# SamsungSAILMontreal/ghn3

Hardware: AMD Instinct MI355X
Metric: predicted-params/sec (GHN fwd+bwd), ghn3xlm16, 256-node graphs (higher is better)
Workload: dtype f16; 1 GPU; ghn3xlm16 fwd+bwd, 1 synthetic 256-node graph(s) per GPU (seed 256000+), 86515016 predicted params per GPU, loss = sum of Frobenius norms of the predicted tensors; ghn_params=654365312, decoder_rows=1421, workspace_bytes=2436048640, zero_fill_bytes=2797339192, parallelism=dp1, index_mode=reference, loss=fused into the tile kernels

## Files before the change

### ghn3_amd/csrc/elementwise.hip

```cpp

#include "ghn3_internal.h"

#define MAX_DEGREE 100
#define MAX_INPUT_DIST 1000

__device__ __forceinline__ float wsum(float v) {
#pragma unroll
    for (int o = 32; o > 0; o >>= 1) v += __shfl_xor(v, o, 64);
    return v;
}

static int launch_ok(const char* what) {
    hipError_t e = hipGetLastError();
    if (e != hipSuccess) { ghn3_set_error("%s launch: %s", what, hipGetErrorString(e)); return GHN3_E_HIP; }
    return GHN3_OK;
}

__global__ __launch_bounds__(256) void graph_prologue_kernel(const int64_t* __restrict__ A, int* __restrict__ deg_in,
                                                             int* __restrict__ deg_out, int* __restrict__ dist0,
                                                             int* __restrict__ pair, int N, int V) {
    __shared__ int red[2][4];
    const int i = blockIdx.x, b = blockIdx.y;
    const int64_t* Ab = A + (size_t)b * N * N;
    int cnt_out = 0, cnt_in = 0;
// ... 450 lines not shown
                    const int c = lane + 64 * j;
                    pv[p][j] = (p < n_add && c < C) ? ar[p * add_stride + c] : 0.f;
                }
#pragma unroll
            for (int p = 0; p < LN_PLANES; ++p)
#pragma unroll
                for (int j = 0; j < LN_REG; ++j) dgv[j] += pv[p][j];
            for (int p = LN_PLANES; p < n_add; ++p)
                for (int j = 0; j < LN_REG; ++j) { const int c = lane + 64 * j; if (c < C) dgv[j] += ar[p * add_stride + c]; }
#pragma unroll
            for (int j = 0; j < LN_REG; ++j) { const int c = lane + 64 * j; if (c < C) gr[c] = dgv[j]; }
        }
#pragma unroll
        for (int j = 0; j < LN_REG; ++j) { const int c = lane + 64 * j; dgv[j] *= (c < C) ? g[c] : 0.f; }
        float s1 = 0.f, s2 = 0.f;
#pragma unroll
        for (int j = 0; j < LN_REG; ++j)
            if (lane + 64 * j < C) {
                s1 += dgv[j];
                s2 += dgv[j] * (xh[j] - mu) * rs;
            }
        s1 = wsum(s1) / (float)C;
        s2 = wsum(s2) / (float)C;
#pragma unroll
        for (int j = 0; j < LN_REG; ++j) {
            const int c = lane + 64 * j;
            if (c < C) {
                const float h = (xh[j] - mu) * rs;
                float v = rs * (dgv[j] - s1 - h * s2);
                if (rr) v += rv[j];
                dr[c] = v;
            }
        }
        return;
    }
    if (ar)
        for (int c = lane; c < C; c += 64) {
            float v = gr[c];
            for (int p = 0; p < n_add; ++p) v += ar[p * add_stride + c];
            gr[c] = v;
        }
    float s1 = 0.f, s2 = 0.f;
    for (int c = lane; c < C; c += 64) {
        const float dg = gr[c] * g[c];
        s1 += dg;
        s2 += dg * (xr[c] - mu) * rs;
    }
    s1 = wsum(s1) / (float)C;
    s2 = wsum(s2) / (float)C;
    for (int c = lane; c < C; c += 64) {
        const float xh = (xr[c] - mu) * rs;
        float v = rs * (gr[c] * g[c] - s1 - xh * s2);
        if (rr) v += rr[c];
        dr[c] = v;
    }
}
int ghn3_layernorm_bwd(float* dx, float* dy, const float* x, const float* g, const float* mean,
                       const float* rstd, const float* res, const float* add, int n_add, int64_t add_stride, int rows,
                       int C, hipStream_t s) {
    if (add && n_add <= 0) n_add = 1;
    hipLaunchKernelGGL(layernorm_bwd_kernel, dim3((rows + 3) / 4), dim3(256), 0, s, dx, dy, x, g, mean, rstd, res, add,
                       n_add, add_stride, rows, C);
    return launch_ok("layernorm_bwd");
}

__global__ __launch_bounds__(256) void ln_param_grad_kernel(float* __restrict__ dg, float* __restrict__ db,
                                                            const float* __restrict__ dy, const float* __restrict__ x,
                                                            const float* __restrict__ mean,
                                                            const float* __restrict__ rstd, int rows, int C, int accum) {
    __shared__ float sg[16][16], sb[16][16];
    const int cl = threadIdx.x & 15, rl = threadIdx.x >> 4;
    const int c = blockIdx.x * 16 + cl;
    float ag = 0.f, ab = 0.f;
    if (c < C) {
        for (int r0 = rl; r0 < rows; r0 += 16 * 8) {
            float d[8], xv[8], mu[8], rs[8];
#pragma unroll
            for (int k = 0; k < 8; ++k) {
                const int r = r0 + 16 * k;
                const bool in = r < rows;
                d[k] = in ? dy[(size_t)r * C + c] : 0.f;
                xv[k] = in ? x[(size_t)r * C + c] : 0.f;
                mu[k] = in ? mean[r] : 0.f;
                rs[k] = in ? rstd[r] : 0.f;
            }
#pragma unroll
            for (int k = 0; k < 8; ++k) { ag += d[k] * (xv[k] - mu[k]) * rs[k]; ab += d[k]; }
        }
    }
    sg[rl][cl] = ag; sb[rl][cl] = ab;
    __syncthreads();
    if (rl == 0 && c < C) {
        float g = 0.f, b = 0.f;
#pragma unroll
        for (int k = 0; k < 16; ++k) { g += sg[k][cl]; b += sb[k][cl]; }
        dg[c] = accum ? dg[c] + g : g;
        db[c] = accum ? db[c] + b : b;
    }
}
__global__ __launch_bounds__(256) void ln_param_grad_batch_kernel(float* __restrict__ gbase, const float* __restrict__ abase,
                                                                  const int64_t* __restrict__ table, int rows, int C) {
    __shared__ float sg[16][16], sb[16][16];
    const int64_t* T = table + 6 * (int64_t)blockIdx.y;
    float* dg = gbase + T[0];
    float* db = gbase + T[1];
    const float* dy = abase + T[2];
    const float* x = abase + T[3];
    const float* mean = abase + T[4];
    const float* rstd = abase + T[5];
    const int cl = threadIdx.x & 15, rl = threadIdx.x >> 4;
    const int c = blockIdx.x * 16 + cl;
    float ag = 0.f, ab = 0.f;
    if (c < C) {
        for (int r0 = rl; r0 < rows; r0 += 16 * 8) {
            float d[8], xv[8], mu[8], rs[8];
#pragma unroll
            for (int k = 0; k < 8; ++k) {
                const int r = r0 + 16 * k;
                const bool in = r < rows;
                d[k] = in ? dy[(size_t)r * C + c] : 0.f;
                xv[k] = in ? x[(size_t)r * C + c] : 0.f;
                mu[k] = in ? mean[r] : 0.f;
                rs[k] = in ? rstd[r] : 0.f;
            }
#pragma unroll
            for (int k = 0; k < 8; ++k) { ag += d[k] * (xv[k] - mu[k]) * rs[k]; ab += d[k]; }
        }
    }
    sg[rl][cl] = ag; sb[rl][cl] = ab;
    __syncthreads();
    if (rl == 0 && c < C) {
        float g = 0.f, b = 0.f;
#pragma unroll
        for (int k = 0; k < 16; ++k) { g += sg[k][cl]; b += sb[k][cl]; }
        dg[c] += g;
        db[c] += b;
    }
}
int ghn3_ln_param_grad_batch(float* gbase, const float* abase, const int64_t* table, int n_items, int rows, int C,
                             hipStream_t s) {
    if (n_items <= 0 || rows <= 0 || C <= 0) return GHN3_OK;
    hipLaunchKernelGGL(ln_param_grad_batch_kernel, dim3((C + 15) / 16, n_items), dim3(256), 0, s, gbase, abase, table, rows, C);
    return launch_ok("ln_param_grad_batch");
}

int ghn3_ln_param_grad(float* dg, float* db, const float* dy, const float* x, const float* mean, const float* rstd,
                       int rows, int C, int accum, hipStream_t s) {
    hipLaunchKernelGGL(ln_param_grad_kernel, dim3((C + 15) / 16), dim3(256), 0, s, dg, db, dy, x, mean, rstd, rows, C,
                       accum);
    return launch_ok("ln_param_grad");
}

struct RowSet { int64_t off; int32_t rows, o, i, ld, i0, _pad; };
__global__ __launch_bounds__(256) void rowset_colsum_kernel(float* __restrict__ out, const float* __restrict__ X,
                                                            const RowSet* __restrict__ sets, int n_sets, int I) {
    __shared__ float red[4][64];
    const int l = threadIdx.x & 63, rl = threadIdx.x >> 6;
    const int ip = blockIdx.x * 64 + l, op = blockIdx.y;
    float acc = 0.f;
    for (int k = 0; k < n_sets; ++k) {
        const RowSet S = sets[k];
        const int il = ip - S.i0;
        if (op >= S.o || (int)(blockIdx.x * 64 + 63) < S.i0 || (int)(blockIdx.x * 64) >= S.i0 + S.i) continue;
        if (il >= 0 && il < S.i) {
            const float* p = X + S.off + (size_t)op * S.i + il;
            for (int r0 = rl; r0 < S.rows; r0 += 4 * 8) {
                float v[8];
#pragma unroll
                for (int e = 0; e < 8; ++e) { const int r = r0 + 4 * e; v[e] = r < S.rows ? p[(size_t)r * S.ld] : 0.f; }
#pragma unroll
                for (int e = 0; e < 8; ++e) acc += v[e];
            }
        }
    }
    red[rl][l] = acc;
    __syncthreads();
    if (rl == 0 && ip < I) out[(size_t)op * I + ip] += (red[0][l] + red[1][l]) + (red[2][l] + red[3][l]);
}
int ghn3_rowset_colsum(float* out, const float* X, const void* sets, int n_sets, int O, int I, hipStream_t s) {
    if (n_sets <= 0 || O <= 0 || I <= 0) return GHN3_OK;
    hipLaunchKernelGGL(rowset_colsum_kernel, dim3((I + 63) / 64, O), dim3(256), 0, s, out, X,
                       reinterpret_cast<const RowSet*>(sets), n_sets, I);
    return launch_ok("rowset_colsum");
}

#define TILE_CHUNK 2048

__device__ __forceinline__ float norm_apply(float v, int mode, float scale) {
    if (mode == 0) return v * scale;
    if (mode == 1) return 2.f / (1.f + __expf(-0.5f * v));
    return tanhf(0.2f * v);
}
__device__ __forceinline__ float norm_grad(float v, int mode, float scale) {
    if (mode == 0) return scale;
    if (mode == 1) { float sg = 1.f / (1.f + __expf(-0.5f * v)); return sg * (1.f - sg); }
    float th = tanhf(0.2f * v);
    return 0.2f * (1.f - th * th);
}

typedef float f4u __attribute__((ext_vector_type(4), aligned(4)));
typedef unsigned short us4h __attribute__((ext_vector_type(4)));
struct SrcTable { const float* p[6]; };
struct DstTable { float* p[6]; };

struct Odo {
    int d[4];
    int T[4];
    int s[4];
    __device__ __forceinline__ void init(unsigned e, unsigned stride, int t0, int t1, int t2, int t3) {
        T[0] = t0; T[1] = t1; T[2] = t2; T[3] = t3;
        unsigned q = e;
        d[3] = q % t3; q /= t3; d[2] = q % t2; q /= t2; d[1] = q % t1; d[0] = q / t1;
        q = stride;
        s[3] = q % t3; q /= t3; s[2] = q % t2; q /= t2; s[1] = q % t1; s[0] = q / t1;
    }
    __device__ __forceinline__ void step() {
        int c = 0;
#pragma unroll
        for (int k = 3; k >= 1; --k) {
            int v = d[k] + s[k] + c;
            c = v >= T[k];
            d[k] = c ? v - T[k] : v;
        }
        d[0] += s[0] + c;
    }
};

__device__ __forceinline__ void tile_block_sumsq(float ss, float bm, float* __restrict__ sq_parts, float* __restrict__ b_parts,
                                                 const ghn3_tile_desc* __restrict__ D) {
    __shared__ float sq_red[4], mx_red[4];
    ss = wsum(ss);
#pragma unroll
    for (int o = 32; o > 0; o >>= 1) bm = fmaxf(bm, __shfl_xor(bm, o, 64));
    __syncthreads();
    if ((threadIdx.x & 63) == 0) { sq_red[threadIdx.x >> 6] = ss; mx_red[threadIdx.x >> 6] = bm; }
    __syncthreads();
    if (threadIdx.x == 0) {
        sq_parts[blockIdx.x] = (sq_red[0] + sq_red[1]) + (sq_red[2] + sq_red[3]);
        if (b_parts) {
            float f = 0.f;
            if (D->src_buf == 0 && D->mode == 0) {
                f = fabsf(D->scale);
#pragma unroll
                for (int k = 0; k < 4; ++k) f *= (float)((D->T[k] + D->E[k] - 1) / D->E[k]);
            }
            b_parts[blockIdx.x] = fmaxf(fmaxf(mx_red[0], mx_red[1]), fmaxf(mx_red[2], mx_red[3])) * f;
        }
    }
}

__global__ __launch_bounds__(256) void tile_fwd_kernel(float* __restrict__ flat, SrcTable srcs,
                                                       const ghn3_tile_desc* __restrict__ desc,
                                                       const int64_t* __restrict__ blocks, float* __restrict__ sq_parts,
                                                       float* __restrict__ b_parts) {
    extern __shared__ float tl[];
    float ss = 0.f, bm = 0.f;
    const int64_t di_raw = blocks[2 * (size_t)blockIdx.x];
    if (di_raw < 0) {
        const ghn3_tile_desc* D = desc + (~di_raw);
        const int64_t word = blocks[2 * (size_t)blockIdx.x + 1];
        const int a0 = (int)(word & 0xffffff), i0 = (int)(word >> 24);
        const int T1 = D->T[1], T3 = D->T[3], hw = D->T[2] * T3, E1 = D->E[1];
        const int ni = min(D->_pad, T1 - i0);
        const float* src = srcs.p[D->src_buf] + D->src_off + (int64_t)(a0 % D->E[0]) * D->S[0];
        const int n = ni * hw;
        const int S2 = (int)D->S[2], S3 = (int)D->S[3];
        const float inv_ni = 1.f / (float)ni, inv_t3 = 1.f / (float)T3;
        const bool vec = E1 == T1 && (ni & 3) == 0 && (S2 & 3) == 0 && (S3 & 3) == 0 &&
                         ((reinterpret_cast<uintptr_t>(src + i0)) & 15) == 0;
        if (vec) {
            const int ni4 = ni >> 2, n4 = ni4 * hw;
            const float inv_ni4 = 1.f / (float)ni4;
            constexpr int U = 4;
            for (int b0 = threadIdx.x; b0 < n4; b0 += 256 * U) {
                float4 v[U];
                int li[U];
#pragma unroll
                for (int u = 0; u < U; ++u) {
                    const int idx = b0 + 256 * u;
                    int pp = (int)((float)idx * inv_ni4);
                    int i4 = idx - pp * ni4;
                    if (i4 < 0) { i4 += ni4; --pp; } else if (i4 >= ni4) { i4 -= ni4; ++pp; }
                    int y = (int)((float)pp * inv_t3);
                    int x = pp - y * T3;
                    if (x < 0) { x += T3; --y; } else if (x >= T3) { x -= T3; ++y; }
                    li[u] = i4 * 4 * hw + pp;
                    v[u] = idx < n4 ? *reinterpret_cast<const float4*>(src + (int64_t)y * S2 + (int64_t)x * S3 + i0 + i4 * 4)
                                    : make_float4(0.f, 0.f, 0.f, 0.f);
                }
#pragma unroll
                for (int u = 0; u < U; ++u)
                    if (b0 + 256 * u < n4) {
                        tl[li[u]] = v[u].x; tl[li[u] + hw] = v[u].y; tl[li[u] + 2 * hw] = v[u].z; tl[li[u] + 3 * hw] = v[u].w;
                    }
            }
        } else {
            constexpr int U = 8;
            for (int b0 = threadIdx.x; b0 < n; b0 += 256 * U) {
                float v[U];
                int li[U];
#pragma unroll
                for (int u = 0; u < U; ++u) {
                    const int idx = b0 + 256 * u;
                    int pp = (int)((float)idx * inv_ni);
                    int i = idx - pp * ni;
                    if (i < 0) { i += ni; --pp; } else if (i >= ni) { i -= ni; ++pp; }
                    int y = (int)((float)pp * inv_t3);
                    int x = pp - y * T3;
                    if (x < 0) { x += T3; --y; } else if (x >= T3) { x -= T3; ++y; }
                    li[u] = i * hw + pp;
                    const int si = i0 + i;
                    v[u] = idx < n ? src[(int64_t)y * S2 + (int64_t)x * S3 + (E1 == T1 ? si : si % E1)] : 0.f;
                }
#pragma unroll
                for (int u = 0; u < U; ++u)
                    if (b0 + 256 * u < n) tl[li[u]] = v[u];
            }
        }
        __syncthreads();
        float* dst = flat + D->dst_off + ((int64_t)a0 * T1 + i0) * hw;
        const float scale = D->scale;
        const int nv = n & ~3;
        for (int j = threadIdx.x * 4; j < nv; j += 1024) {
            f4u o;
            o.x = tl[j] * scale; o.y = tl[j + 1] * scale; o.z = tl[j + 2] * scale; o.w = tl[j + 3] * scale;
            *reinterpret_cast<f4u*>(dst + j) = o;
            ss += (o.x * o.x + o.y * o.y) + (o.z * o.z + o.w * o.w);
            bm = fmaxf(fmaxf(bm, fmaxf(fabsf(o.x), fabsf(o.y))), fmaxf(fabsf(o.z), fabsf(o.w)));
        }
        for (int j = nv + threadIdx.x; j < n; j += 256) { const float o = tl[j] * scale; dst[j] = o; ss += o * o; bm = fmaxf(bm, fabsf(o)); }
        if (sq_parts) tile_block_sumsq(ss, bm, sq_parts, b_parts, D);
        return;
    }
    const int64_t di = di_raw;
    const unsigned start = (unsigned)blocks[2 * (size_t)blockIdx.x + 1];
// ... 702 lines not shown
                    const float4 v = *reinterpret_cast<const float4*>(p);
                    acc[0] += v.x; acc[1] += v.y; acc[2] += v.z; acc[3] += v.w;
                } else for (int k = 0; k < cnt; ++k) acc[k] += p[k];
            }
        }
        for (int k = 0; k < cnt; ++k) {
            if (OUT16) reinterpret_cast<unsigned short*>(out_)[e + k] = wire_bf16(acc[k] * scale);
            else reinterpret_cast<float*>(out_)[e + k] = acc[k] * scale;
        }
    }
}
int ghn3_rank_reduce(void* out, const void* in, int64_t per, int W, int in16, int out16, float scale, hipStream_t s) {
    if (per <= 0 || W <= 0) return GHN3_OK;
    int64_t blocks = (per / 4 + 255) / 256 + 1;
    if (blocks > 8192) blocks = 8192;
    const dim3 g((unsigned)blocks), b(256);
    if (in16 && out16) hipLaunchKernelGGL((rank_reduce_kernel<true, true>), g, b, 0, s, out, in, per, W, scale);
    else if (in16) hipLaunchKernelGGL((rank_reduce_kernel<true, false>), g, b, 0, s, out, in, per, W, scale);
    else if (out16) hipLaunchKernelGGL((rank_reduce_kernel<false, true>), g, b, 0, s, out, in, per, W, scale);
    else hipLaunchKernelGGL((rank_reduce_kernel<false, false>), g, b, 0, s, out, in, per, W, scale);
    return launch_ok("rank_reduce");
}

__global__ __launch_bounds__(256) void transpose32_kernel(float* __restrict__ dst, const float* __restrict__ src, int rows, int cols,
                                                          int ld_src, int ld_dst, int64_t sb, int64_t db) {
    __shared__ float t[64][65];
    const float* S = src + (int64_t)blockIdx.z * sb;
    float* D = dst + (int64_t)blockIdx.z * db;
    const int r0 = blockIdx.y * 64, c0 = blockIdx.x * 64;
    const int tx = threadIdx.x & 15, ty = threadIdx.x >> 4;
    for (int i = ty; i < 64; i += 16) {
        const int r = r0 + i, c = c0 + tx * 4;
        float4 v = {0.f, 0.f, 0.f, 0.f};
        if (r < rows) {
            if (c + 3 < cols && ((ld_src & 3) == 0) && ((reinterpret_cast<uintptr_t>(S) & 15) == 0)) v = *reinterpret_cast<const float4*>(S + (int64_t)r * ld_src + c);
            else { float e[4] = {0.f, 0.f, 0.f, 0.f}; for (int k = 0; k < 4; ++k) if (c + k < cols) e[k] = S[(int64_t)r * ld_src + c + k]; v = {e[0], e[1], e[2], e[3]}; }
        }
        t[i][tx * 4] = v.x; t[i][tx * 4 + 1] = v.y; t[i][tx * 4 + 2] = v.z; t[i][tx * 4 + 3] = v.w;
    }
    __syncthreads();
    for (int i = ty; i < 64; i += 16) {
        const int c = c0 + i, r = r0 + tx * 4;
        if (c >= cols) continue;
        float e[4] = {t[tx * 4][i], t[tx * 4 + 1][i], t[tx * 4 + 2][i], t[tx * 4 + 3][i]};
        if (r + 3 < rows && ((ld_dst & 3) == 0) && ((reinterpret_cast<uintptr_t>(D) & 15) == 0)) *reinterpret_cast<float4*>(D + (int64_t)c * ld_dst + r) = float4{e[0], e[1], e[2], e[3]};
        else for (int k = 0; k < 4; ++k) if (r + k < rows) D[(int64_t)c * ld_dst + r + k] = e[k];
    }
}
int ghn3_transpose32(float* dst, const float* src, int rows, int cols, int ld_src, int ld_dst, int batch, int64_t sb, int64_t db,
                     hipStream_t s) {
    if (rows <= 0 || cols <= 0 || batch <= 0) return GHN3_OK;
    if (batch > 65535 || (rows + 63) / 64 > 65535) { ghn3_set_error("transpose32: too many batches / row tiles"); return GHN3_E_LIMIT; }
    hipLaunchKernelGGL(transpose32_kernel, dim3((cols + 63) / 64, (rows + 63) / 64, batch), dim3(256), 0, s, dst, src, rows, cols,
                       ld_src, ld_dst, sb, db);
    return launch_ok("transpose32");
}

__device__ __forceinline__ unsigned short cast_f16(float x) {
    const float c = x != x ? x : __builtin_amdgcn_fmed3f(x, -65504.f, 65504.f);
    return __builtin_bit_cast(unsigned short, (_Float16)c);
}
__device__ __forceinline__ unsigned short cast_bf16(float x) {
    unsigned u = __builtin_bit_cast(unsigned, x);
    u += 0x7fffu + ((u >> 16) & 1u);
    return (unsigned short)(u >> 16);
}
__device__ __forceinline__ float bf16_back(unsigned short h) { return __builtin_bit_cast(float, (unsigned)h << 16); }
__device__ __forceinline__ float f16_back(unsigned short h) { return (float)__builtin_bit_cast(_Float16, h); }
typedef unsigned short us4 __attribute__((ext_vector_type(4)));
typedef unsigned short us8 __attribute__((ext_vector_type(8)));

struct AdamWArgs { float lr, beta1, beta2, eps, weight_decay, bias_corr1, bias_corr2_sqrt, max_norm, inv_scale; int nt; };
typedef float f32x4_nt __attribute__((ext_vector_type(4)));
__device__ __forceinline__ float4 ld4(const float* p, bool nt) {
    if (nt) { const f32x4_nt v = __builtin_nontemporal_load(reinterpret_cast<const f32x4_nt*>(p)); return make_float4(v[0], v[1], v[2], v[3]); }
    return *reinterpret_cast<const float4*>(p);
}
__device__ __forceinline__ void st4(float* p, const float4& x, bool nt) {
    if (nt) { const f32x4_nt v = {x.x, x.y, x.z, x.w}; __builtin_nontemporal_store(v, reinterpret_cast<f32x4_nt*>(p)); }
    else *reinterpret_cast<float4*>(p) = x;
}
static int adamw_nt_env() {
    static const int v = getenv("GHN3_ADAMW_NT") ? atoi(getenv("GHN3_ADAMW_NT")) != 0 : 1;
    return v;
}
template <typename MT> struct AdamWSrcT { const float* g; MT* m; MT* v; const float* sumsq; AdamWArgs a; };
typedef AdamWSrcT<float> AdamWSrc;

struct AdamWRng { unsigned key; unsigned base; };
__host__ __device__ __forceinline__ unsigned adamw_mix32(unsigned x) {
    x ^= x >> 16; x *= 0x7feb352du; x ^= x >> 15; x *= 0x846ca68bu; x ^= x >> 16;
    return x;
}
static unsigned adamw_rng_key(unsigned seed, unsigned step) { return adamw_mix32(seed * 0x9e3779b9u + step); }
__device__ __forceinline__ unsigned short bf16_stochastic(float x, unsigned r16) {
    return (unsigned short)((__builtin_bit_cast(unsigned, x) + r16) >> 16);
}
typedef unsigned u32x2_nt __attribute__((ext_vector_type(2)));
template <int NT> __device__ __forceinline__ float4 ld_m4(const float* p, bool nt) { return ld4(p, nt); }
template <int NT> __device__ __forceinline__ float4 ld_m4(const unsigned short* p, bool) {
    u32x2_nt w;
    if constexpr (NT > 0) w = __builtin_nontemporal_load(reinterpret_cast<const u32x2_nt*>(p));
    else w = *reinterpret_cast<const u32x2_nt*>(p);
    return make_float4(__builtin_bit_cast(float, w[0] << 16), __builtin_bit_cast(float, w[0] & 0xffff0000u),
                       __builtin_bit_cast(float, w[1] << 16), __builtin_bit_cast(float, w[1] & 0xffff0000u));
}
template <int NT>
__device__ __forceinline__ void st_mv4(float* m, float* v, const float4& mv, const float4& vv, bool nt, const AdamWRng&, unsigned) {
    st4(m, mv, nt); st4(v, vv, nt);
}
template <int NT>
__device__ __forceinline__ void st_mv4(unsigned short* m, unsigned short* v, const float4& mv, const float4& vv, bool,
                                       const AdamWRng& rng, unsigned idx) {
    const unsigned h0 = adamw_mix32(idx ^ rng.key), h1 = adamw_mix32((idx + 1u) ^ rng.key),
                   h2 = adamw_mix32((idx + 2u) ^ rng.key), h3 = adamw_mix32((idx + 3u) ^ rng.key);
    const u32x2_nt wm = {(unsigned)bf16_stochastic(mv.x, h0 & 0xffffu) | ((unsigned)bf16_stochastic(mv.y, h1 & 0xffffu) << 16),
                         (unsigned)bf16_stochastic(mv.z, h2 & 0xffffu) | ((unsigned)bf16_stochastic(mv.w, h3 & 0xffffu) << 16)};
    const u32x2_nt wv = {(unsigned)bf16_stochastic(vv.x, h0 >> 16) | ((unsigned)bf16_stochastic(vv.y, h1 >> 16) << 16),
                         (unsigned)bf16_stochastic(vv.z, h2 >> 16) | ((unsigned)bf16_stochastic(vv.w, h3 >> 16) << 16)};
    if constexpr (NT > 0) {
        __builtin_nontemporal_store(wm, reinterpret_cast<u32x2_nt*>(m));
        __builtin_nontemporal_store(wv, reinterpret_cast<u32x2_nt*>(v));
    } else {
        *reinterpret_cast<u32x2_nt*>(m) = wm;
        *reinterpret_cast<u32x2_nt*>(v) = wv;
    }
}
__device__ __forceinline__ float ld_m1(const float* p) { return *p; }
__device__ __forceinline__ float ld_m1(const unsigned short* p) { return bf16_back(*p); }
__device__ __forceinline__ void st_mv1(float* m, float* v, float mi, float vi, const AdamWRng&, unsigned) { *m = mi; *v = vi; }
__device__ __forceinline__ void st_mv1(unsigned short* m, unsigned short* v, float mi, float vi, const AdamWRng& rng, unsigned idx) {
    const unsigned h = adamw_mix32(idx ^ rng.key);
    *m = bf16_stochastic(mi, h & 0xffffu); *v = bf16_stochastic(vi, h >> 16);
}

__device__ __forceinline__ float nofuse(float x) { asm volatile("" : "+v"(x)); return x; }
__device__ __forceinline__ void adamw_scalars(const AdamWArgs& a, const float* sumsq, float& clip, float& step, float& decay) {
    clip = a.inv_scale;
    if (sumsq && a.max_norm > 0.f)
        clip = clip * fminf(1.f, a.max_norm / (nofuse(sqrtf(*sumsq) * a.inv_scale) + 1e-6f));
    step = a.lr / a.bias_corr1;
    decay = 1.f - nofuse(a.lr * a.weight_decay);
}
__device__ __forceinline__ void adamw_element(float& p, float g, float& m, float& v, const AdamWArgs& a, float clip,
                                              float step, float decay) {
    const float gi = g * clip;
    const float mi = __builtin_fmaf(a.beta1, m, nofuse((1.f - a.beta1) * gi));
    const float vi = __builtin_fmaf(a.beta2, v, nofuse(nofuse((1.f - a.beta2) * gi) * gi));
    m = mi; v = vi;
    const float den = nofuse(sqrtf(vi) / a.bias_corr2_sqrt) + a.eps;
    p = nofuse(p * decay) - nofuse(nofuse(step * mi) / den);
}

template <bool ADAMW, typename MT = float, int NT = -1>
__device__ __forceinline__ void cast16_body(const float* __restrict__ src, unsigned short* __restrict__ dst,
                                            const ghn3_cast_desc* __restrict__ descs, int n_desc,
                                            float* __restrict__ dbias, int total_items,
                                            const float* __restrict__ amax, const AdamWSrcT<MT>& aw,
                                            const AdamWRng& rng = AdamWRng{}) {
    __shared__ unsigned short tr[64][66];
    __shared__ float csum[16][64];
    float aw_clip = 1.f, aw_step = 0.f, aw_decay = 1.f;
    if (ADAMW) {
        if (aw.sumsq && !isfinite(*aw.sumsq)) return;
        adamw_scalars(aw.a, aw.sumsq, aw_clip, aw_step, aw_decay);
    }
    for (int item = blockIdx.x; item < total_items; item += gridDim.x) {
    int lo = 0, hi = n_desc - 1;
    while (lo < hi) {
        const int mid = (lo + hi + 1) >> 1;
        if (descs[mid].block_start <= item) lo = mid; else hi = mid - 1;
    }
    const ghn3_cast_desc D = descs[lo];
    const int t = item - D.block_start;
    const int tiles_c = (D.cols + 63) >> 6;
    const int r0 = (t / tiles_c) * 64, c0 = (t % tiles_c) * 64;
    const int tid = threadIdx.x;
    const int c4 = (tid & 15) * 4, rr = tid >> 4;
    const float* S = src + D.src_off;
    const bool st = D.flags & GHN3_CAST_STRAIGHT, trn = D.flags & GHN3_CAST_TRANSPOSED;
    const bool split = D.flags & GHN3_CAST_SPLIT;
    const bool frag = D.flags & GHN3_CAST_FRAG;
    const bool st_f16s = split && (D.flags & GHN3_CAST_SPLIT_F16);
    const float s16 = st_f16s ? (float)(1 << GHN3_X3F16_WSHIFT) : 1.f;
    const bool st_bf = ((D.flags & GHN3_CAST_STRAIGHT_BF16) || split) && !st_f16s, tr_bf = (D.flags & GHN3_CAST_TRANSPOSED_BF16) || split;
    const float sc = ((D.flags & GHN3_CAST_SCALED) && amax) ? ghn3_pow2_scale(*amax) : 1.f;
    const int rows_w = (D.flags & GHN3_CAST_TIGHT) ? ((D.rows + 7) & ~7) : 0x7fffffff;

    if (!ADAMW && st && !trn && !frag && !(D.flags & (GHN3_CAST_COLSUM | GHN3_CAST_SRC16)) && D.src_q == 0 && !(D.ld_dst & 7) && !(D.dst_off & 7) && !(D.lo_off & 7)) {
        unsigned short* Dd = dst + D.dst_off;
        const int64_t wp = (int64_t)tiles_c * 64;
#pragma unroll
        for (int i = 0; i < 2; ++i) {
            const int64_t e0 = (int64_t)t * 4096 + 2048 * i + tid * 8;
            const int r = (int)(e0 / wp), c = (int)(e0 - (int64_t)r * wp);
            if (r >= D.rows) continue;
            const float* p = S + (int64_t)r * D.ld_src + c;
            float x[8];
            if (c + 7 < D.cols) {
                const float4 a = *reinterpret_cast<const float4*>(p), b = *reinterpret_cast<const float4*>(p + 4);
                x[0] = a.x; x[1] = a.y; x[2] = a.z; x[3] = a.w; x[4] = b.x; x[5] = b.y; x[6] = b.z; x[7] = b.w;
            } else {
#pragma unroll
                for (int e = 0; e < 8; ++e) x[e] = c + e < D.cols ? p[e] : 0.f;
            }
            us8 h, l;
#pragma unroll
            for (int e = 0; e < 8; ++e) {
                const float xs = x[e] * sc * s16;
                h[e] = st_bf ? cast_bf16(xs) : cast_f16(xs);
                if (split) l[e] = st_f16s ? cast_f16(xs - f16_back(h[e])) : cast_bf16(xs - bf16_back(h[e]));
            }
            *reinterpret_cast<us8*>(Dd + (int64_t)r * D.ld_dst + c) = h;
            if (split) *reinterpret_cast<us8*>(Dd + D.lo_off + (int64_t)r * D.ld_dst + c) = l;
        }
        continue;
    }
    const bool src16 = D.flags & GHN3_CAST_SRC16;
    float4 v[4];
#pragma unroll
    for (int i = 0; i < 4; ++i) {
        const int r = r0 + rr + 16 * i, c = c0 + c4;
        float4 x = make_float4(0.f, 0.f, 0.f, 0.f);
        if (r < D.rows) {
            const int sc_ = D.src_q > 0 ? (c / D.src_q) * D.src_s + c % D.src_q : c;
            if (src16) {
                const unsigned short* p = dst + D.src_off + (int64_t)r * D.ld_src + sc_;
                unsigned short h0 = 0, h1 = 0, h2 = 0, h3 = 0;
                if (c + 3 < D.cols) {
                    const uint2 w = *reinterpret_cast<const uint2*>(p);
                    h0 = (unsigned short)(w.x & 0xffffu); h1 = (unsigned short)(w.x >> 16);
                    h2 = (unsigned short)(w.y & 0xffffu); h3 = (unsigned short)(w.y >> 16);
                } else {
                    if (c < D.cols) h0 = p[0];
                    if (c + 1 < D.cols) h1 = p[1];
                    if (c + 2 < D.cols) h2 = p[2];
                }
                if (tr_bf) x = make_float4(bf16_back(h0), bf16_back(h1), bf16_back(h2), bf16_back(h3));
                else x = make_float4(f16_back(h0), f16_back(h1), f16_back(h2), f16_back(h3));
            } else if (ADAMW) {
                if (c + 3 < D.cols) {
                    const int64_t o = D.src_off + (int64_t)r * D.ld_src + c;
                    float* pp = const_cast<float*>(src) + o;
                    const bool nt = NT < 0 ? aw.a.nt != 0 : NT != 0;
                    x = ld4(pp, nt);
                    const float4 gv = ld4(aw.g + o, nt);
                    float4 mv = ld_m4<NT>(aw.m + o, nt), vv = ld_m4<NT>(aw.v + o, nt);
                    adamw_element(x.x, gv.x, mv.x, vv.x, aw.a, aw_clip, aw_step, aw_decay);
                    adamw_element(x.y, gv.y, mv.y, vv.y, aw.a, aw_clip, aw_step, aw_decay);
                    adamw_element(x.z, gv.z, mv.z, vv.z, aw.a, aw_clip, aw_step, aw_decay);
                    adamw_element(x.w, gv.w, mv.w, vv.w, aw.a, aw_clip, aw_step, aw_decay);
                    st_mv4<NT>(aw.m + o, aw.v + o, mv, vv, nt, rng, rng.base + (unsigned)o);
                    st4(pp, x, nt);
                }
            } else {
                const float* p = S + (int64_t)r * D.ld_src + sc_;
                if (c + 3 < D.cols) x = *reinterpret_cast<const float4*>(p);
                else {
                    if (c < D.cols) x.x = p[0];
                    if (c + 1 < D.cols) x.y = p[1];
                    if (c + 2 < D.cols) x.z = p[2];
                }
            }
        }
        v[i] = x;
    }
    if (D.flags & GHN3_CAST_COLSUM) {
        const float un = src16 ? 1.f / sc : 1.f;
        csum[rr][c4] = (v[0].x + v[1].x + v[2].x + v[3].x) * un;
        csum[rr][c4 + 1] = (v[0].y + v[1].y + v[2].y + v[3].y) * un;
        csum[rr][c4 + 2] = (v[0].z + v[1].z + v[2].z + v[3].z) * un;
        csum[rr][c4 + 3] = (v[0].w + v[1].w + v[2].w + v[3].w) * un;
    }
    if (sc != 1.f && !src16) {
#pragma unroll
        for (int i = 0; i < 4; ++i) { v[i].x *= sc; v[i].y *= sc; v[i].z *= sc; v[i].w *= sc; }
    }
    if (st) {
        unsigned short* Dd = dst + D.dst_off;
#pragma unroll
        for (int i = 0; i < 4; ++i) {
            const int r = r0 + rr + 16 * i;
            if (r >= D.rows) continue;
            us4 h;
            const float4 vs = make_float4(v[i].x * s16, v[i].y * s16, v[i].z * s16, v[i].w * s16);
            if (st_bf) { h[0] = cast_bf16(v[i].x); h[1] = cast_bf16(v[i].y); h[2] = cast_bf16(v[i].z); h[3] = cast_bf16(v[i].w); }
            else { h[0] = cast_f16(vs.x); h[1] = cast_f16(vs.y); h[2] = cast_f16(vs.z); h[3] = cast_f16(vs.w); }
            const int c = c0 + c4;
            const int64_t o = frag ? ((int64_t)(r >> 4) * (D.cols >> 5) + (c >> 5)) * 512 + ((((c & 31) >> 3) * 16 + (r & 15)) << 3) + (c & 7)
                                   : (int64_t)r * D.ld_dst + c;
            if (frag && c >= D.cols) continue;
            *reinterpret_cast<us4*>(Dd + o) = h;
            if (split) {
                us4 l;
                if (st_f16s) {
                    l[0] = cast_f16(vs.x - f16_back(h[0])); l[1] = cast_f16(vs.y - f16_back(h[1]));
                    l[2] = cast_f16(vs.z - f16_back(h[2])); l[3] = cast_f16(vs.w - f16_back(h[3]));
                } else {
                    l[0] = cast_bf16(v[i].x - bf16_back(h[0])); l[1] = cast_bf16(v[i].y - bf16_back(h[1]));
                    l[2] = cast_bf16(v[i].z - bf16_back(h[2])); l[3] = cast_bf16(v[i].w - bf16_back(h[3]));
                }
                *reinterpret_cast<us4*>(Dd + D.lo_off + o) = l;
            }
        }
    }
    if (trn) {
#pragma unroll
        for (int i = 0; i < 4; ++i) {
            const int r = rr + 16 * i;
            if (tr_bf) {
                tr[r][c4] = cast_bf16(v[i].x); tr[r][c4 + 1] = cast_bf16(v[i].y);
                tr[r][c4 + 2] = cast_bf16(v[i].z); tr[r][c4 + 3] = cast_bf16(v[i].w);
            } else {
                tr[r][c4] = cast_f16(v[i].x); tr[r][c4 + 1] = cast_f16(v[i].y);
                tr[r][c4 + 2] = cast_f16(v[i].z); tr[r][c4 + 3] = cast_f16(v[i].w);
            }
        }
    }
    __syncthreads();
    if (trn) {
        unsigned short* Dt = dst + D.dstT_off;
#pragma unroll
        for (int i = 0; i < 2; ++i) {
            const int p = tid + 256 * i;
            const int col = p >> 3, rp = (p & 7) * 8;
            if (c0 + col >= D.cols || r0 + rp >= rows_w) continue;
            us8 h;
#pragma unroll
            for (int e = 0; e < 8; ++e) h[e] = tr[rp + e][col];
            const int fn = c0 + col, fk = r0 + rp;
            const int64_t o = frag ? ((int64_t)(fn >> 4) * (D.rows >> 5) + (fk >> 5)) * 512 + ((((fk & 31) >> 3) * 16 + (fn & 15)) << 3)
                                   : (int64_t)fn * D.ld_dstT + fk;
            if (frag && fk >= D.rows) continue;
            *reinterpret_cast<us8*>(Dt + o) = h;
        }
    }
    if (trn && split) {
        __syncthreads();
#pragma unroll
        for (int i = 0; i < 4; ++i) {
            const int r = rr + 16 * i;
            tr[r][c4] = cast_bf16(v[i].x - bf16_back(cast_bf16(v[i].x)));
            tr[r][c4 + 1] = cast_bf16(v[i].y - bf16_back(cast_bf16(v[i].y)));
            tr[r][c4 + 2] = cast_bf16(v[i].z - bf16_back(cast_bf16(v[i].z)));
            tr[r][c4 + 3] = cast_bf16(v[i].w - bf16_back(cast_bf16(v[i].w)));
        }
        __syncthreads();
        unsigned short* Dt = dst + D.dstT_off + D.lo_off;
#pragma unroll
        for (int i = 0; i < 2; ++i) {
            const int p = tid + 256 * i;
            const int col = p >> 3, rp = (p & 7) * 8;
            if (c0 + col >= D.cols || r0 + rp >= rows_w) continue;
            us8 h;
#pragma unroll
            for (int e = 0; e < 8; ++e) h[e] = tr[rp + e][col];
            const int fn = c0 + col, fk = r0 + rp;
            const int64_t o = frag ? ((int64_t)(fn >> 4) * (D.rows >> 5) + (fk >> 5)) * 512 + ((((fk & 31) >> 3) * 16 + (fn & 15)) << 3)
                                   : (int64_t)fn * D.ld_dstT + fk;
            if (frag && fk >= D.rows) continue;
            *reinterpret_cast<us8*>(Dt + o) = h;
        }
    }
    if ((D.flags & GHN3_CAST_COLSUM) && tid < 64 && c0 + tid < D.cols) {
        float s = 0.f;
#pragma unroll
        for (int w = 0; w < 16; ++w) s += csum[w][tid];
        if (D.flags & GHN3_CAST_COLSUM_PARTS) {
            dbias[D.part_off + (int64_t)(r0 >> 6) * D.cols + c0 + tid] = s;
        } else {
            int c = c0 + tid;
            if (D.bias_q > 0) c = (c / D.bias_q) * D.bias_s + c % D.bias_q;
            atomicAdd(dbias + c + D.bias_off, s);
        }
    }
    __syncthreads();
    }
}

__global__ __launch_bounds__(256) void cast16_kernel(const float* __restrict__ src, unsigned short* __restrict__ dst,
                                                     const ghn3_cast_desc* __restrict__ descs, int n_desc,
                                                     float* __restrict__ dbias, int total_items,
                                                     const float* __restrict__ amax) {
    cast16_body<false>(src, dst, descs, n_desc, dbias, total_items, amax, AdamWSrc{});
}
__global__ __launch_bounds__(256) void adamw_cast16_kernel(float* __restrict__ p, unsigned short* __restrict__ dst,
                                                           const ghn3_cast_desc* __restrict__ descs, int n_desc,
                                                           int total_items, AdamWSrc aw) {
    cast16_body<true>(p, dst, descs, n_desc, nullptr, total_items, nullptr, aw);
}
template <int NT>
__global__ __launch_bounds__(256) void adamw_s16_cast16_kernel(float* __restrict__ p, unsigned short* __restrict__ dst,
                                                               const ghn3_cast_desc* __restrict__ descs, int n_desc,
                                                               int total_items, AdamWSrcT<unsigned short> aw, AdamWRng rng) {
    cast16_body<true, unsigned short, NT>(p, dst, descs, n_desc, nullptr, total_items, nullptr, aw, rng);
}

int ghn3_cast16(const float* src, void* dst, const ghn3_cast_desc* d_desc, int n_desc, int total_blocks, float* dbias,
                const float* amax, int grid_cap, hipStream_t s) {
    if (n_desc <= 0 || total_blocks <= 0) return GHN3_OK;
    const int grid = grid_cap > 0 && grid_cap < total_blocks ? grid_cap : total_blocks;
    hipLaunchKernelGGL(cast16_kernel, dim3(grid), dim3(256), 0, s, src, (unsigned short*)dst, d_desc, n_desc,
                       dbias, total_blocks, amax);
    return launch_ok("cast16");
}

__global__ __launch_bounds__(256) void sumsq_kernel(float* __restrict__ out, const float* __restrict__ x, int64_t n,
                                                    float* __restrict__ parts) {
    __shared__ float part[4];
    float acc = 0.f;
    const int64_t n4 = n >> 2;
    const float4* x4 = reinterpret_cast<const float4*>(x);
    for (int64_t i = (int64_t)blockIdx.x * 256 + threadIdx.x; i < n4; i += (int64_t)gridDim.x * 256) {
        const float4 v = x4[i];
        acc += v.x * v.x + v.y * v.y + v.z * v.z + v.w * v.w;
    }
    if (blockIdx.x == 0 && threadIdx.x < (n & 3)) { const float v = x[(n4 << 2) + threadIdx.x]; acc += v * v; }
#pragma unroll
    for (int o = 32; o > 0; o >>= 1) acc += __shfl_xor(acc, o, 64);
    if ((threadIdx.x & 63) == 0) part[threadIdx.x >> 6] = acc;
    __syncthreads();
    if (threadIdx.x == 0) {
        const float t = (part[0] + part[1]) + (part[2] + part[3]);
        if (parts) parts[blockIdx.x] = t; else atomicAdd(out, t);
    }
}
__global__ void sumsq_finish_kernel(float* __restrict__ out, const float* __restrict__ parts, int n) {
    __shared__ float tot[256];
    float acc = 0.f;
    for (int k = threadIdx.x; k < n; k += 256) acc += parts[k];
    tot[threadIdx.x] = acc;
    __syncthreads();
    if (threadIdx.x == 0) { float t = 0.f; for (int k = 0; k < 256; ++k) t += tot[k]; out[0] += t; }
}
__global__ __launch_bounds__(256) void slot_sum_kernel(float* __restrict__ parts, const float* __restrict__ x, int n) {
    __shared__ float part[4];
    float a0 = 0.f, a1 = 0.f, a2 = 0.f, a3 = 0.f;
    const int n4 = n >> 2;
    const float4* x4 = reinterpret_cast<const float4*>(x);
    for (int i = blockIdx.x * 256 + threadIdx.x; i < n4; i += gridDim.x * 256) {
        const float4 v = x4[i];
        a0 += v.x; a1 += v.y; a2 += v.z; a3 += v.w;
    }
    float acc = (a0 + a1) + (a2 + a3);
    if (blockIdx.x == 0 && threadIdx.x < (n & 3)) acc += x[(n4 << 2) + threadIdx.x];
#pragma unroll
    for (int o = 32; o > 0; o >>= 1) acc += __shfl_xor(acc, o, 64);
    if ((threadIdx.x & 63) == 0) part[threadIdx.x >> 6] = acc;
    __syncthreads();
    if (threadIdx.x == 0) parts[blockIdx.x] = (part[0] + part[1]) + (part[2] + part[3]);
}
int ghn3_sumsq(float* out, const float* x, int64_t n, float* parts, int64_t skip_lo, int64_t skip_hi, const float* extra,
               int n_extra, hipStream_t s) {
    if (n <= 0) return GHN3_OK;
    if (reinterpret_cast<uintptr_t>(x) & 15) { ghn3_set_error("sumsq: buffer must be 16-byte aligned"); return GHN3_E_ARG; }
    const bool skip = skip_hi > skip_lo;
    if (skip || n_extra > 0) {
        if (!parts || skip_lo < 0 || skip_hi > n || (skip_lo & 3) || (skip_hi & 3) || (n_extra > 0 && !extra)) {
            ghn3_set_error("sumsq: a skipped range needs the scratch buffer, 4-float alignment and 0 <= lo <= hi <= n");
            return GHN3_E_ARG;
        }
    }
    auto blocks_of = [](int64_t m) { int64_t b = (m / 4 + 255) / 256; return (int)(b < 1 ? 1 : (b > 4096 ? 4096 : b)); };
    if (!skip && n_extra <= 0) {
        const int blocks = blocks_of(n);
        hipLaunchKernelGGL(sumsq_kernel, dim3(blocks), dim3(256), 0, s, out, x, n, parts);
        if (parts) hipLaunchKernelGGL(sumsq_finish_kernel, dim3(1), dim3(256), 0, s, out, parts, blocks);
        return launch_ok("sumsq");
    }
    int b0 = 0, b1 = 0, b2 = 0;
    const int64_t lo = skip ? skip_lo : n, hi = skip ? skip_hi : n;
    if (lo > 0) {
        b0 = blocks_of(lo);
        hipLaunchKernelGGL(sumsq_kernel, dim3(b0), dim3(256), 0, s, out, x, lo, parts);
    }
    if (n > hi) {
        b1 = blocks_of(n - hi);
        if (b1 > 4032) b1 = 4032;
        hipLaunchKernelGGL(sumsq_kernel, dim3(b1), dim3(256), 0, s, out, x + hi, n - hi, parts + b0);
    }
    if (n_extra > 0) {
        if (reinterpret_cast<uintptr_t>(extra) & 15) { ghn3_set_error("sumsq: slot table must be 16-byte aligned"); return GHN3_E_ARG; }
        b2 = 64;
        hipLaunchKernelGGL(slot_sum_kernel, dim3(b2), dim3(256), 0, s, parts + b0 + b1, extra, n_extra);
    }
    hipLaunchKernelGGL(sumsq_finish_kernel, dim3(1), dim3(256), 0, s, out, parts, b0 + b1 + b2);
    return launch_ok("sumsq");
}

template <typename MT, int NT = -1>
__device__ __forceinline__ void adamw_body(float* __restrict__ p, const float* __restrict__ g,
                                           MT* __restrict__ m, MT* __restrict__ v, int64_t n,
                                           const float* __restrict__ sumsq, const AdamWArgs& a, const AdamWRng& rng) {
    if (sumsq && !isfinite(*sumsq)) return;
    float clip, step, decay;
    adamw_scalars(a, sumsq, clip, step, decay);
    int64_t n4 = 0;
    constexpr uintptr_t MA = 4 * sizeof(MT) - 1;
    if (((reinterpret_cast<uintptr_t>(p) | reinterpret_cast<uintptr_t>(g)) & 15) == 0 &&
        ((reinterpret_cast<uintptr_t>(m) | reinterpret_cast<uintptr_t>(v)) & MA) == 0) {
        n4 = n >> 2;
        const bool nt = NT < 0 ? a.nt != 0 : NT != 0;
        for (int64_t i = (int64_t)blockIdx.x * 256 + threadIdx.x; i < n4; i += (int64_t)gridDim.x * 256) {
            float4 pv = ld4(p + 4 * i, nt), gv = ld4(g + 4 * i, nt), mv = ld_m4<NT>(m + 4 * i, nt), vv = ld_m4<NT>(v + 4 * i, nt);
            float* pe = &pv.x; float* ge = &gv.x; float* me = &mv.x; float* ve = &vv.x;
#pragma unroll
            for (int e = 0; e < 4; ++e) adamw_element(pe[e], ge[e], me[e], ve[e], a, clip, step, decay);
            st_mv4<NT>(m + 4 * i, v + 4 * i, mv, vv, nt, rng, rng.base + (unsigned)(4 * i)); st4(p + 4 * i, pv, nt);
        }
    }
    for (int64_t i = 4 * n4 + (int64_t)blockIdx.x * 256 + threadIdx.x; i < n; i += (int64_t)gridDim.x * 256) {
        float pi = p[i], mi = ld_m1(m + i), vi = ld_m1(v + i);
        adamw_element(pi, g[i], mi, vi, a, clip, step, decay);
        st_mv1(m + i, v + i, mi, vi, rng, rng.base + (unsigned)i); p[i] = pi;
    }
}
__global__ __launch_bounds__(256) void adamw_kernel(float* __restrict__ p, const float* __restrict__ g,
                                                    float* __restrict__ m, float* __restrict__ v, int64_t n,
                                                    const float* __restrict__ sumsq, AdamWArgs a) {
    adamw_body<float>(p, g, m, v, n, sumsq, a, AdamWRng{});
}
template <int NT>
__global__ __launch_bounds__(256) void adamw_s16_kernel(float* __restrict__ p, const float* __restrict__ g,
                                                        unsigned short* __restrict__ m, unsigned short* __restrict__ v,
                                                        int64_t n, const float* __restrict__ sumsq, AdamWArgs a, AdamWRng rng) {
    adamw_body<unsigned short, NT>(p, g, m, v, n, sumsq, a, rng);
}
int ghn3_adamw_cast16(float* p, const float* g, float* m, float* v, void* dst, const ghn3_cast_desc* d_desc, int n_desc,
                      int total_blocks, const float* sumsq, float lr, float beta1, float beta2, float eps, float weight_decay,
                      float bias_corr1, float bias_corr2, float max_norm, float inv_scale, hipStream_t s) {
    if (n_desc <= 0 || total_blocks <= 0) return GHN3_OK;
    if ((reinterpret_cast<uintptr_t>(p) | reinterpret_cast<uintptr_t>(g) | reinterpret_cast<uintptr_t>(m) |
         reinterpret_cast<uintptr_t>(v)) & 15) {
        ghn3_set_error("adamw_cast16: buffers must be 16-byte aligned");
        return GHN3_E_ARG;
    }
    AdamWSrc aw{g, m, v, sumsq, AdamWArgs{lr, beta1, beta2, eps, weight_decay, bias_corr1, sqrtf(bias_corr2), max_norm,
                                           inv_scale > 0.f ? inv_scale : 1.f, adamw_nt_env()}};
    hipLaunchKernelGGL(adamw_cast16_kernel, dim3(total_blocks), dim3(256), 0, s, p, (unsigned short*)dst, d_desc, n_desc,
                       total_blocks, aw);
    return launch_ok("adamw_cast16");
}

int ghn3_adamw(float* p, const float* g, float* m, float* v, int64_t n, const float* sumsq, float lr, float beta1,
               float beta2, float eps, float weight_decay, float bias_corr1, float bias_corr2, float max_norm,
               float inv_scale, hipStream_t s) {
    if (n <= 0) return GHN3_OK;
    AdamWArgs a{lr, beta1, beta2, eps, weight_decay, bias_corr1, sqrtf(bias_corr2), max_norm,
                inv_scale > 0.f ? inv_scale : 1.f, adamw_nt_env()};
    int64_t blocks = (n / 4 + 255) / 256 + 1;
    if (blocks > 16384) blocks = 16384;
    hipLaunchKernelGGL(adamw_kernel, dim3((unsigned)blocks), dim3(256), 0, s, p, g, m, v, n, sumsq, a);
    return launch_ok("adamw");
}
// ... 54 lines not shown
```

Baseline: 15.29 billion predicted-params/s.

## Add vectorized relayout cast16 path and streaming rowset colsum kernel

Adds a cast16 variant that handles f16-source transposed relayout descriptors with 128-row tiles, vectorized 8/4-wide loads, a swizzled LDS image and 16-byte transposed stores. Descriptor lookup becomes a wave-ballot search instead of a per-item binary search. The rowset column-sum gets a streaming kernel that precomputes segment lists in LDS, processes four output rows per block and issues batched float4 loads. This targets memory inefficiency in the transpose/colsum passes, at the cost of more LDS use, extra code paths and fallbacks for unaligned cases. Both paths are enabled by default and can be turned off with an environment variable.

```diff
diff --git a/ghn3_amd/csrc/elementwise.hip b/ghn3_amd/csrc/elementwise.hip
--- a/ghn3_amd/csrc/elementwise.hip
+++ b/ghn3_amd/csrc/elementwise.hip
@@ -626,11 +626,15 @@
 }
 
 struct RowSet { int64_t off; int32_t rows, o, i, ld, i0, _pad; };
-__global__ __launch_bounds__(256) void rowset_colsum_kernel(float* __restrict__ out, const float* __restrict__ X,
-                                                            const RowSet* __restrict__ sets, int n_sets, int I) {
-    __shared__ float red[4][64];
+static bool relayout16_on() {
+    static const int v = getenv("GHN3_RELAYOUT16") ? atoi(getenv("GHN3_RELAYOUT16")) != 0 : 1;
+    return v != 0;
+}
+__device__ __forceinline__ void rowset_colsum_block(float* __restrict__ out, const float* __restrict__ X,
+                                                    const RowSet* __restrict__ sets, int n_sets, int I, int op,
+                                                    float (*red)[64]) {
     const int l = threadIdx.x & 63, rl = threadIdx.x >> 6;
-    const int ip = blockIdx.x * 64 + l, op = blockIdx.y;
+    const int ip = blockIdx.x * 64 + l;
     float acc = 0.f;
     for (int k = 0; k < n_sets; ++k) {
         const RowSet S = sets[k];
@@ -651,10 +655,99 @@
     __syncthreads();
     if (rl == 0 && ip < I) out[(size_t)op * I + ip] += (red[0][l] + red[1][l]) + (red[2][l] + red[3][l]);
 }
+__global__ __launch_bounds__(256) void rowset_colsum_kernel(float* __restrict__ out, const float* __restrict__ X,
+                                                            const RowSet* __restrict__ sets, int n_sets, int I) {
+    __shared__ float red[4][64];
+    rowset_colsum_block(out, X, sets, n_sets, I, blockIdx.y, red);
+}
+
+constexpr int kRowsetSegCap = 512, kRowsetBatch = 8;
+__global__ __launch_bounds__(256) void rowset_colsum_stream_kernel(float* __restrict__ out, const float* __restrict__ X,
+                                                                   const RowSet* __restrict__ sets, int n_sets, int O, int I) {
+    __shared__ float red[4][4][64];
+    __shared__ int nseg[256];
+    __shared__ int4 seg_a[kRowsetSegCap], seg_b[kRowsetSegCap];
+    __shared__ int total_s;
+    const int tid = threadIdx.x, cb = blockIdx.x * 64, op0 = blockIdx.y * 4;
+    int total = kRowsetSegCap + 1;
+    if (n_sets <= 256) {
+        int ns = 0, unaligned = 0;
+        RowSet S = {};
+        if (tid < n_sets) {
+            S = sets[tid];
+            const bool hit = S.rows > 0 && S.i > 0 && op0 < S.o && cb + 63 >= S.i0 && cb < S.i0 + S.i;
+            ns = hit ? (S.rows + 7) >> 3 : 0;
+            if (ns > kRowsetSegCap) ns = kRowsetSegCap + 1;
+            unaligned = hit && ((((int)S.off | S.i | S.ld | S.i0) & 3) != 0);
+        }
+        nseg[tid] = ns;
+        unaligned = __syncthreads_or(unaligned);
+        int at = 0;
+        for (int j = 0; j < tid && j < n_sets; ++j) at += nseg[j];
+        if (tid == n_sets - 1) total_s = at + ns;
+        if (at + ns <= kRowsetSegCap)
+            for (int sgi = 0; sgi < ns; ++sgi) {
+                seg_a[at + sgi] = make_int4((int)(S.off & 0xffffffffll), (int)(S.off >> 32), S.rows, S.o);
+                seg_b[at + sgi] = make_int4(S.i, S.ld, S.i0, sgi * 8);
+            }
+        __syncthreads();
+        total = unaligned ? kRowsetSegCap + 1 : total_s;
+    }
+    if (total > kRowsetSegCap) {
+        for (int w = 0; w < 4 && op0 + w < O; ++w) {
+            rowset_colsum_block(out, X, sets, n_sets, I, op0 + w, red[0]);
+            __syncthreads();
+        }
+        return;
+    }
+    const int w = tid >> 6, lane = tid & 63, q = lane & 15, rl = lane >> 4;
+    const int op = op0 + w, ipq = cb + 4 * q;
+    float4 acc = make_float4(0.f, 0.f, 0.f, 0.f);
+    for (int n0 = 0; n0 < total && op < O; n0 += kRowsetBatch) {
+        int4 sa[kRowsetBatch], sb[kRowsetBatch];
+        float4 va[kRowsetBatch], vb[kRowsetBatch];
+        bool ina[kRowsetBatch], inb[kRowsetBatch];
+#pragma unroll
+        for (int u = 0; u < kRowsetBatch; ++u) {
+            const int n = n0 + u < total ? n0 + u : total - 1;
+            sa[u] = seg_a[n];
+            sb[u] = seg_b[n];
+        }
+#pragma unroll
+        for (int u = 0; u < kRowsetBatch; ++u) {
+            const int64_t off = (int64_t)(((uint64_t)(unsigned)sa[u].y << 32) | (unsigned)sa[u].x);
+            const int rows = sa[u].z, o = sa[u].w, i = sb[u].x, ld = sb[u].y, i0 = sb[u].z;
+            const int ra = sb[u].w + rl, rb = ra + 4;
+            const int il = ipq - i0;
+            const bool in = n0 + u < total && op < o && il >= 0 && il < i;
+            const int opc = op < o ? op : o - 1, ilc = il < 0 ? 0 : (il < i ? il : i - 4);
+            const float* p = X + off + (size_t)opc * i + ilc;
+            va[u] = *reinterpret_cast<const float4*>(p + (size_t)(ra < rows ? ra : rows - 1) * ld);
+            vb[u] = *reinterpret_cast<const float4*>(p + (size_t)(rb < rows ? rb : rows - 1) * ld);
+            ina[u] = in && ra < rows;
+            inb[u] = in && rb < rows;
+        }
+#pragma unroll
+        for (int u = 0; u < kRowsetBatch; ++u) {
+            const float4 a = ina[u] ? va[u] : make_float4(0.f, 0.f, 0.f, 0.f), b = inb[u] ? vb[u] : make_float4(0.f, 0.f, 0.f, 0.f);
+            acc.x += a.x; acc.y += a.y; acc.z += a.z; acc.w += a.w;
+            acc.x += b.x; acc.y += b.y; acc.z += b.z; acc.w += b.w;
+        }
+    }
+    *reinterpret_cast<float4*>(&red[w][rl][4 * q]) = acc;
+    __syncthreads();
+    const int ip = cb + lane;
+    if (op < O && ip < I)
+        out[(size_t)op * I + ip] += (red[w][0][lane] + red[w][1][lane]) + (red[w][2][lane] + red[w][3][lane]);
+}
 int ghn3_rowset_colsum(float* out, const float* X, const void* sets, int n_sets, int O, int I, hipStream_t s) {
     if (n_sets <= 0 || O <= 0 || I <= 0) return GHN3_OK;
-    hipLaunchKernelGGL(rowset_colsum_kernel, dim3((I + 63) / 64, O), dim3(256), 0, s, out, X,
-                       reinterpret_cast<const RowSet*>(sets), n_sets, I);
+    if (relayout16_on() && (reinterpret_cast<uintptr_t>(X) & 15) == 0)
+        hipLaunchKernelGGL(rowset_colsum_stream_kernel, dim3((I + 63) / 64, (O + 3) / 4), dim3(256), 0, s, out, X,
+                           reinterpret_cast<const RowSet*>(sets), n_sets, O, I);
+    else
+        hipLaunchKernelGGL(rowset_colsum_kernel, dim3((I + 63) / 64, O), dim3(256), 0, s, out, X,
+                           reinterpret_cast<const RowSet*>(sets), n_sets, I);
     return launch_ok("rowset_colsum");
 }
 
@@ -1663,27 +1756,161 @@
     p = nofuse(p * decay) - nofuse(nofuse(step * mi) / den);
 }
 
-template <bool ADAMW, typename MT = float, int NT = -1>
+constexpr int kRelayoutLds = 64 * 128;
+__device__ __forceinline__ bool cast16_is_relayout(unsigned flags) {
+    return (flags & (GHN3_CAST_SRC16 | GHN3_CAST_TRANSPOSED)) == (GHN3_CAST_SRC16 | GHN3_CAST_TRANSPOSED) &&
+           !(flags & (GHN3_CAST_STRAIGHT | GHN3_CAST_SPLIT | GHN3_CAST_FRAG));
+}
+__device__ __forceinline__ void cast16_relayout_tile(const ghn3_cast_desc& D, int t, unsigned short* __restrict__ dst,
+                                                     float* __restrict__ dbias, const float* __restrict__ amax,
+                                                     unsigned short* __restrict__ img, float (*csum)[64]) {
+    const int tiles_c = (D.cols + 63) >> 6, tiles_r = (D.rows + 63) >> 6;
+    if (t >= ((tiles_r + 1) >> 1) * tiles_c) return;
+    const int r0 = (t / tiles_c) * 128, c0 = (t % tiles_c) * 64;
+    const int tid = threadIdx.x;
+    const int cq = tid & 7, rr = (tid >> 3) & 15, half = tid >> 7;
+    const int c = c0 + cq * 8;
+    const unsigned short* __restrict__ S = dst + D.src_off;
+    const int q = D.src_q, s = D.src_s;
+    const bool al4 = (((int)D.src_off | D.ld_src | q | s) & 3) == 0 && (reinterpret_cast<uintptr_t>(dst) & 7) == 0;
+    const bool al8 = (((int)D.src_off | D.ld_src | q | s) & 7) == 0 && (reinterpret_cast<uintptr_t>(dst) & 15) == 0;
+    const int vec = (al8 && D.cols >= 8) ? 8 : (al4 && D.cols >= 4) ? 4 : 0;
+    us8 x[4];
+    if (vec == 8) {
+        const bool cin = c + 8 <= D.cols;
+        const int cs = cin ? (q > 0 ? (c / q) * s + c % q : c) : 0;
+#pragma unroll
+        for (int i = 0; i < 4; ++i) {
+            const int r = r0 + half * 64 + rr + 16 * i;
+            const us8 w = *reinterpret_cast<const us8*>(S + (int64_t)(r < D.rows ? r : D.rows - 1) * D.ld_src + cs);
+            x[i] = (cin && r < D.rows) ? w : us8(0);
+        }
+    } else if (vec == 4) {
+        const bool cin0 = c + 4 <= D.cols, cin1 = c + 8 <= D.cols;
+        const int cs0 = cin0 ? (q > 0 ? (c / q) * s + c % q : c) : 0;
+        const int cs1 = cin1 ? (q > 0 ? ((c + 4) / q) * s + (c + 4) % q : c + 4) : 0;
+#pragma unroll
+        for (int i = 0; i < 4; ++i) {
+            const int r = r0 + half * 64 + rr + 16 * i;
+            const unsigned short* p = S + (int64_t)(r < D.rows ? r : D.rows - 1) * D.ld_src;
+            const us4 w0 = *reinterpret_cast<const us4*>(p + cs0), w1 = *reinterpret_cast<const us4*>(p + cs1);
+            const us4 z0 = (cin0 && r < D.rows) ? w0 : us4(0), z1 = (cin1 && r < D.rows) ? w1 : us4(0);
+            x[i] = us8{z0[0], z0[1], z0[2], z0[3], z1[0], z1[1], z1[2], z1[3]};
+        }
+    } else {
+#pragma unroll
+        for (int i = 0; i < 4; ++i) x[i] = us8(0);
+    }
+    if (vec == 0 || c0 + 64 > D.cols) {
+#pragma unroll
+        for (int i = 0; i < 4; ++i) {
+            const int r = r0 + half * 64 + rr + 16 * i;
+#pragma unroll
+            for (int e = 0; e < 8; ++e) {
+                const int ce = c + e;
+                const bool covered = vec == 8 ? c + 8 <= D.cols : vec == 4 ? c + (e & 4) + 4 <= D.cols : false;
+                if (!covered && r < D.rows && ce < D.cols)
+                    x[i][e] = S[(int64_t)r * D.ld_src + (q > 0 ? (ce / q) * s + ce % q : ce)];
+            }
+        }
+    }
+    const bool bf = D.flags & GHN3_CAST_TRANSPOSED_BF16;
+    if (D.flags & GHN3_CAST_COLSUM) {
+        const float sc = ((D.flags & GHN3_CAST_SCALED) && amax) ? ghn3_pow2_scale(*amax) : 1.f;
+        const float un = 1.f / sc;
+#pragma unroll
+        for (int e = 0; e < 8; ++e) {
+            const float v0 = bf ? bf16_back(x[0][e]) : f16_back(x[0][e]), v1 = bf ? bf16_back(x[1][e]) : f16_back(x[1][e]),
+                        v2 = bf ? bf16_back(x[2][e]) : f16_back(x[2][e]), v3 = bf ? bf16_back(x[3][e]) : f16_back(x[3][e]);
+            csum[half * 16 + rr][cq * 8 + e] = (v0 + v1 + v2 + v3) * un;
+        }
+    }
+#pragma unroll
+    for (int i = 0; i < 4; ++i) {
+        const int k = half * 64 + rr + 16 * i;
+#pragma unroll
+        for (int e = 0; e < 8; ++e) img[(cq * 8 + e) * 128 + ((((k >> 3) ^ cq) & 15) << 3) + (k & 7)] = x[i][e];
+    }
+    __syncthreads();
+    if ((D.flags & GHN3_CAST_COLSUM) && tid < 128) {
+        const int hf = tid >> 6, col = tid & 63;
+        if (c0 + col < D.cols && r0 + hf * 64 < D.rows) {
+            float sum = 0.f;
+#pragma unroll
+            for (int w = 0; w < 16; ++w) sum += csum[hf * 16 + w][col];
+            if (D.flags & GHN3_CAST_COLSUM_PARTS) {
+                dbias[D.part_off + (int64_t)((r0 >> 6) + hf) * D.cols + c0 + col] = sum;
+            } else {
+                int cb = c0 + col;
+                if (D.bias_q > 0) cb = (cb / D.bias_q) * D.bias_s + cb % D.bias_q;
+                atomicAdd(dbias + cb + D.bias_off, sum);
+            }
+        }
+    }
+    const int k_end = (D.flags & GHN3_CAST_TIGHT) ? ((D.rows + 7) & ~7) : ((D.rows + 63) & ~63);
+    unsigned short* __restrict__ Dt = dst + D.dstT_off;
+#pragma unroll
+    for (int i = 0; i < 4; ++i) {
+        const int p = tid + 256 * i;
+        const int col = p >> 4, j = p & 15;
+        const us8 h = *reinterpret_cast<const us8*>(img + col * 128 + (((j ^ (col >> 3)) & 15) << 3));
+        if (c0 + col < D.cols && r0 + 8 * j < k_end)
+            *reinterpret_cast<us8*>(Dt + (int64_t)(c0 + col) * D.ld_dstT + r0 + 8 * j) = h;
+    }
+    __syncthreads();
+}
+
+template <bool WAVE> struct Cast16Starts {
+    int bs[4];
+    __device__ __forceinline__ Cast16Starts(const ghn3_cast_desc* __restrict__ descs, int n_desc) {
+        if (WAVE && n_desc <= 256) {
+#pragma unroll
+            for (int j = 0; j < 4; ++j) {
+                const int k = j * 64 + (int)(threadIdx.x & 63);
+                bs[j] = descs[k < n_desc ? k : n_desc - 1].block_start;
+                if (k >= n_desc) bs[j] = 0x7fffffff;
+            }
+        }
+    }
+    __device__ __forceinline__ int find(const ghn3_cast_desc* __restrict__ descs, int n_desc, int item) const {
+        if (WAVE && n_desc <= 256) {
+            int cnt = 0;
+#pragma unroll
+            for (int j = 0; j < 4; ++j) cnt += __popcll(__ballot(bs[j] <= item));
+            return __builtin_amdgcn_readfirstlane(cnt > 0 ? cnt - 1 : 0);
+        }
+        int lo = 0, hi = n_desc - 1;
+        while (lo < hi) {
+            const int mid = (lo + hi + 1) >> 1;
+            if (descs[mid].block_start <= item) lo = mid; else hi = mid - 1;
+        }
+        return lo;
+    }
+};
+
+template <bool ADAMW, typename MT = float, int NT = -1, bool RELAYOUT = false>
 __device__ __forceinline__ void cast16_body(const float* __restrict__ src, unsigned short* __restrict__ dst,
                                             const ghn3_cast_desc* __restrict__ descs, int n_desc,
                                             float* __restrict__ dbias, int total_items,
                                             const float* __restrict__ amax, const AdamWSrcT<MT>& aw,
                                             const AdamWRng& rng = AdamWRng{}) {
-    __shared__ unsigned short tr[64][66];
-    __shared__ float csum[16][64];
+    __shared__ __attribute__((aligned(16))) unsigned short tr_img[RELAYOUT ? kRelayoutLds : 64 * 66];
+    unsigned short (*tr)[66] = reinterpret_cast<unsigned short (*)[66]>(tr_img);
+    __shared__ float csum[RELAYOUT ? 32 : 16][64];
     float aw_clip = 1.f, aw_step = 0.f, aw_decay = 1.f;
     if (ADAMW) {
         if (aw.sumsq && !isfinite(*aw.sumsq)) return;
         adamw_scalars(aw.a, aw.sumsq, aw_clip, aw_step, aw_decay);
     }
+    const Cast16Starts<RELAYOUT> starts(descs, n_desc);
     for (int item = blockIdx.x; item < total_items; item += gridDim.x) {
-    int lo = 0, hi = n_desc - 1;
-    while (lo < hi) {
-        const int mid = (lo + hi + 1) >> 1;
-        if (descs[mid].block_start <= item) lo = mid; else hi = mid - 1;
-    }
+    const int lo = starts.find(descs, n_desc, item);
     const ghn3_cast_desc D = descs[lo];
     const int t = item - D.block_start;
+    if (RELAYOUT && cast16_is_relayout(D.flags)) {
+        cast16_relayout_tile(D, t, dst, dbias, amax, tr_img, csum);
+        continue;
+    }
     const int tiles_c = (D.cols + 63) >> 6;
     const int r0 = (t / tiles_c) * 64, c0 = (t % tiles_c) * 64;
     const int tid = threadIdx.x;
@@ -1895,6 +2122,12 @@
                                                      const float* __restrict__ amax) {
     cast16_body<false>(src, dst, descs, n_desc, dbias, total_items, amax, AdamWSrc{});
 }
+__global__ __launch_bounds__(256, 6) void cast16_relayout_kernel(const float* __restrict__ src, unsigned short* __restrict__ dst,
+                                                              const ghn3_cast_desc* __restrict__ descs, int n_desc,
+                                                              float* __restrict__ dbias, int total_items,
+                                                              const float* __restrict__ amax) {
+    cast16_body<false, float, -1, true>(src, dst, descs, n_desc, dbias, total_items, amax, AdamWSrc{});
+}
 __global__ __launch_bounds__(256) void adamw_cast16_kernel(float* __restrict__ p, unsigned short* __restrict__ dst,
                                                            const ghn3_cast_desc* __restrict__ descs, int n_desc,
                                                            int total_items, AdamWSrc aw) {
@@ -1911,6 +2144,11 @@
                 const float* amax, int grid_cap, hipStream_t s) {
     if (n_desc <= 0 || total_blocks <= 0) return GHN3_OK;
     const int grid = grid_cap > 0 && grid_cap < total_blocks ? grid_cap : total_blocks;
+    if (relayout16_on()) {
+        hipLaunchKernelGGL(cast16_relayout_kernel, dim3(grid), dim3(256), 0, s, src, (unsigned short*)dst, d_desc, n_desc,
+                           dbias, total_blocks, amax);
+        return launch_ok("cast16");
+    }
     hipLaunchKernelGGL(cast16_kernel, dim3(grid), dim3(256), 0, s, src, (unsigned short*)dst, d_desc, n_desc,
                        dbias, total_blocks, amax);
     return launch_ok("cast16");
```

After: 15.41 billion predicted-params/s, median of 6. About the same (+0.8%).
